# ModelTC/Dipoorlet

Hardware: AMD Instinct MI355X
Metric: calibration images/sec (whole node) + achieved HBM GB/s, ResNet-50 ONNX N=1024, -A hist (higher is better)
Workload: dtype f32; 1 GPU; ResNet-50 ONNX activation set (T=123, 26598376 fp32 elems/img), -A hist --bins 2048, N=1024 per GPU in 32 batches of 32: range pass + histogram pass + percentile clip; device=AMD Radeon Graphics (gfx950:sramecc+:xnack-), hist_checksum_ok=True, world_size_seen_by_backend=1

## Files before the change

### dipoorlet_amd/csrc/calib_kernels.hip

```cpp
#include "common.hpp"

#pragma clang fp contract(off)

namespace {

struct MinMaxOp {
    float mn, mx;
    uint32_t nan;
    __device__ __forceinline__ void operator()(float x) {
        mn = fminf(mn, x);
        mx = fmaxf(mx, x);
        nan |= (x != x);
    }
};

__device__ __forceinline__ void minmax_commit(const MinMaxOp& op, uint32_t slot, float* s_mn, float* s_mx, uint32_t* s_nan,
                                              uint32_t* __restrict__ min_enc, uint32_t* __restrict__ max_enc,
                                              uint32_t* __restrict__ nan_flag) {
    float mn = wave_min(op.mn), mx = wave_max(op.mx);
    uint32_t nn = __any(op.nan) ? 1u : 0u;
    const int w = threadIdx.x / kWave;
    if ((threadIdx.x & (kWave - 1)) == 0) {
        s_mn[w] = mn;
        s_mx[w] = mx;
        s_nan[w] = nn;
    }
    __syncthreads();
    if (threadIdx.x == 0) {
#pragma unroll
        for (int j = 1; j < kBlock / kWave; ++j) {
            mn = fminf(mn, s_mn[j]);
            mx = fmaxf(mx, s_mx[j]);
            nn |= s_nan[j];
        }
        if (mn <= mx) {
            atomicMin(min_enc + slot, enc_f32(mn));
            atomicMax(max_enc + slot, enc_f32(mx));
        }
        if (nn) atomicOr(nan_flag + slot, 1u);
    }
    __syncthreads();
}

__global__ __launch_bounds__(kBlock) void k_minmax(const dpl_work_item* __restrict__ items,
                                                    const uint32_t* __restrict__ bb,
                                                    const float* const* __restrict__ segs,
                                                    uint32_t* __restrict__ min_enc, uint32_t* __restrict__ max_enc,
                                                    uint32_t* __restrict__ nan_flag) {
    __shared__ float s_mn[kBlock / kWave], s_mx[kBlock / kWave];
    __shared__ uint32_t s_nan[kBlock / kWave];
    uint32_t k0, k1;
    block_items(bb, k0, k1);
    for (uint32_t k = k0; k < k1; ++k) {
        const dpl_work_item it = items[k];
        MinMaxOp op{INFINITY, -INFINITY, 0u};
        stream_span(segs[it.seg] + it.offset, it.count, op);
        minmax_commit(op, it.slot, s_mn, s_mx, s_nan, min_enc, max_enc, nan_flag);
    }
}

__global__ void k_minmax_init(uint32_t* mn, uint32_t* mx, uint32_t* nan, int64_t n) {
    int64_t i = (int64_t)blockIdx.x * blockDim.x + threadIdx.x;
    if (i < n) {
        mn[i] = 0xFFFFFFFFu;
        mx[i] = 0u;
        nan[i] = 0u;
    }
}

__device__ __forceinline__ void minmax_decode(uint32_t mn, uint32_t mx, uint32_t nan, float& omn, float& omx) {
    const bool bad = nan != 0u || mn == 0xFFFFFFFFu;
    omn = bad ? NAN : dec_f32(mn);
    omx = bad ? NAN : dec_f32(mx);
}

__global__ void k_minmax_finalize(const uint32_t* mn, const uint32_t* mx, const uint32_t* nan, int64_t n,
                                  float* omn, float* omx) {
    int64_t i = (int64_t)blockIdx.x * blockDim.x + threadIdx.x;
    if (i < n) minmax_decode(mn[i], mx[i], nan[i], omn[i], omx[i]);
}

__global__ void k_minmax_encode(const float* mn, const float* mx, int64_t n, uint32_t* emn, uint32_t* emx,
                                uint32_t* nan) {
    int64_t i = (int64_t)blockIdx.x * blockDim.x + threadIdx.x;
    if (i < n) {
        const bool bad = (mn[i] != mn[i]) || (mx[i] != mx[i]);
        emn[i] = bad ? 0xFFFFFFFFu : enc_f32(mn[i]);
        emx[i] = bad ? 0u : enc_f32(mx[i]);
        nan[i] = bad ? 1u : 0u;
    }
}

__device__ __forceinline__ float hist_edge(int i, float step, float first) {
    return __fadd_rn(__fmul_rn((float)i, step), first);
}

template <bool kFast>
struct HistOp {
    uint32_t* lds;
    float first, last, step, inv, denom;
    int last_bin;
    float fbins;
    uint32_t nonzero;
    __device__ __forceinline__ void operator()(float x) {
        const float a = fabsf(x);
        const bool nz = (a != 0.0f);
        nonzero += nz;
        if (kFast) {
            if (nz && (a <= last)) {
                const int i = (int)__fmul_rn(a, inv);
                const uint32_t dec = (a < __fmul_rn((float)i, step)) ? 0xFFFFFFFCu : 0u;
                atomicAdd(reinterpret_cast<uint32_t*>(reinterpret_cast<char*>(lds) + (((uint32_t)i << 2) + dec)), 1u);
            }
            return;
        }
        int i;
        if (kFast) {
            i = (int)__fmul_rn(a, inv);
            i = i > last_bin ? last_bin : i;
            i -= (a < __fmul_rn((float)i, step)) ? 1 : 0;
        } else {
            i = (int)__fmul_rn(__fdiv_rn(__fsub_rn(a, first), denom), fbins);
            i = i > last_bin ? last_bin : i;
            i = i < 0 ? 0 : i;
            i -= (a < hist_edge(i, step, first)) ? 1 : 0;
            i += (i != last_bin && a >= hist_edge(i + 1, step, first)) ? 1 : 0;
        }
        if (nz && (a <= last)) atomicAdd(lds + i, 1u);
    }
};

template <bool kFast>
__device__ __forceinline__ void hist_op_init(HistOp<kFast>& op, const dpl_hist_range& r, int bins, uint32_t* lds) {
    op.lds = lds;
    op.first = r.first;
    op.last = r.last;
    op.step = r.step;
    op.inv = r.inv;
    op.denom = __fsub_rn(r.last, r.first);
    op.last_bin = bins - 1;
    op.fbins = (float)bins;
    op.nonzero = 0u;
}

template <class Count>
__device__ __forceinline__ void hist_flush(uint32_t nonzero, const dpl_work_item& it, const dpl_hist_range& r, int bins,
                                           Count* __restrict__ hist, uint32_t* lds, uint32_t* s_nz) {
    const uint32_t nzw = wave_sum(nonzero);
    if ((threadIdx.x & (kWave - 1)) == 0) s_nz[threadIdx.x / kWave] = nzw;
    __syncthreads();
    if (threadIdx.x == 0) {
        uint32_t nzb = 0;
        for (int k = 0; k < kBlock / kWave; ++k) nzb += s_nz[k];
        const uint32_t z = it.count - nzb;
        if (z) atomicAdd(lds + r.zero_bin, z);
        const uint32_t top = lds[bins];
        if (top) atomicAdd(lds + bins - 1, top);
    }
    __syncthreads();
    Count* __restrict__ out = hist + (uint64_t)it.slot * (uint64_t)bins;
    for (int b = threadIdx.x; b < bins; b += kBlock) {
        const uint32_t c = lds[b];
        if (c) {
            if constexpr (sizeof(Count) == 8)
                atomicAdd(reinterpret_cast<unsigned long long*>(out + b), (unsigned long long)c);
            else
                atomicAdd(out + b, c);
        }
    }
}

template <bool kFast>
__device__ __forceinline__ void hist_body(const dpl_work_item& it, const float* const* __restrict__ segs,
                                          const dpl_hist_range& r, int bins, uint64_t* __restrict__ hist,
                                          uint32_t* lds, uint32_t* s_nz) {
    HistOp<kFast> op;
    hist_op_init(op, r, bins, lds);
    stream_span(segs[it.seg] + it.offset, it.count, op);
    hist_flush(op.nonzero, it, r, bins, hist, lds, s_nz);
}

__global__ __launch_bounds__(kBlock) void k_abs_hist(const dpl_work_item* __restrict__ items,
                                                      const uint32_t* __restrict__ bb,
                                                      const float* const* __restrict__ segs,
                                                      const dpl_hist_range* __restrict__ ranges, int bins,
                                                      uint64_t* __restrict__ hist) {
    extern __shared__ __attribute__((aligned(16))) uint32_t lds[];
    uint32_t* s_nz = lds + bins + 1;
    uint32_t k0, k1;
    block_items(bb, k0, k1);
    for (uint32_t k = k0; k < k1; ++k) {
        const dpl_work_item it = items[k];
        const dpl_hist_range r = ranges[it.slot];
        if (r.status != 0u) continue;
        for (int b = threadIdx.x; b <= bins; b += kBlock) lds[b] = 0u;
        __syncthreads();
        if (r.exact_div)
            hist_body<false>(it, segs, r, bins, hist, lds, s_nz);
        else
            hist_body<true>(it, segs, r, bins, hist, lds, s_nz);
        __syncthreads();
    }
}

__device__ __forceinline__ float py_max(float a, float b) { return (b > a) ? b : a; }
__device__ __forceinline__ float py_min(float a, float b) { return (b < a) ? b : a; }

__device__ __forceinline__ dpl_hist_range hist_range_of(float gmin, float gmax, int bins) {
    dpl_hist_range r;
    const float dmax = py_max(gmax, -gmin);
    float first = 0.0f, last = dmax;
    r.dmax = dmax;
    r.status = 0u;
    if (!(fabsf(last) <= 3.402823466e+38f) || last < first) r.status = 1u;
    if (first == last) {
        first = -0.5f;
        last = 0.5f;
    }
    const float delta = __fsub_rn(last, first);
    const float fb = (float)bins;
    r.first = first;
    r.last = last;
    r.step = __fdiv_rn(delta, fb);
    r.inv = __fmul_rn(__fdiv_rn(fb, delta), 1.000001f);
    if (r.status == 0u) {
        const float e1 = hist_edge(1, r.step, first);
        const float el = hist_edge(bins - 1, r.step, first);
        const float el2 = hist_edge(bins - 2 > 0 ? bins - 2 : 0, r.step, first);
        if (!(r.step > 0.0f) || !(e1 > first) || !(last > el) || (bins > 2 && !(el > el2))) r.status = 2u;
    }
    r.exact_div = (first != 0.0f || !(fabsf(r.inv) <= 3.402823466e+38f) || r.step < 1.0e-30f) ? 1u : 0u;
    {
        const float a = 0.0f;
        float t = __fmul_rn(__fdiv_rn(__fsub_rn(a, first), delta), fb);
        int b = (int)t;
        b = b > bins - 1 ? bins - 1 : b;
        b = b < 0 ? 0 : b;
        if (a < hist_edge(b, r.step, first)) --b;
        if (b != bins - 1 && a >= hist_edge(b + 1, r.step, first)) ++b;
        r.zero_bin = (uint32_t)(b < 0 ? 0 : b);
    }
    return r;
}

__global__ void k_hist_prepare(const float* __restrict__ gmin, const float* __restrict__ gmax, int64_t n, int bins,
                               dpl_hist_range* __restrict__ out) {
    int64_t i = (int64_t)blockIdx.x * blockDim.x + threadIdx.x;
    if (i >= n) return;
    out[i] = hist_range_of(gmin[i], gmax[i], bins);
}

__host__ __device__ inline uint64_t spec_counts_offset(int64_t n_slots) {
    return (((uint64_t)n_slots * (sizeof(dpl_hist_range) + sizeof(uint32_t))) + 15ull) & ~15ull;
}

__global__ __launch_bounds__(kBlock) void k_hist_snapshot(const uint32_t* __restrict__ mn, const uint32_t* __restrict__ mx,
                                                           const uint32_t* __restrict__ nan, int64_t n, int bins,
                                                           dpl_hist_range* __restrict__ snap, uint32_t* __restrict__ flags,
                                                           uint32_t* __restrict__ counts) {
    const int64_t i = (int64_t)blockIdx.x * blockDim.x + threadIdx.x;
    const int64_t stride = (int64_t)gridDim.x * blockDim.x;
    if (i < n) {
        float gmin, gmax;
        minmax_decode(mn[i], mx[i], nan[i], gmin, gmax);
        snap[i] = hist_range_of(gmin, gmax, bins);
        flags[i] = 0u;
    }
    const int64_t total = n * (int64_t)bins;
    for (int64_t j = i; j < total; j += stride) counts[j] = 0u;
}

template <bool kFast>
struct MinMaxHistOp {
    MinMaxOp m;
    HistOp<kFast> h;
    __device__ __forceinline__ void operator()(float x) {
        m(x);
        h(x);
    }
};

template <bool kFast>
__device__ __forceinline__ void minmax_hist_body(const dpl_work_item& it, const float* const* __restrict__ segs,
                                                 const dpl_hist_range& r, int bins, uint32_t* __restrict__ counts,
                                                 uint32_t* lds, uint32_t* s_nz, MinMaxOp& m) {
    MinMaxHistOp<kFast> op;
    op.m = m;
    hist_op_init(op.h, r, bins, lds);
    stream_span(segs[it.seg] + it.offset, it.count, op);
    m = op.m;
    hist_flush(op.h.nonzero, it, r, bins, counts, lds, s_nz);
}

__global__ __launch_bounds__(kBlock) void k_minmax_hist(const dpl_work_item* __restrict__ items,
                                                         const uint32_t* __restrict__ bb,
                                                         const float* const* __restrict__ segs,
                                                         uint32_t* __restrict__ min_enc, uint32_t* __restrict__ max_enc,
                                                         uint32_t* __restrict__ nan_flag,
                                                         const dpl_hist_range* __restrict__ snap, int bins,
                                                         uint32_t* __restrict__ counts) {
    extern __shared__ __attribute__((aligned(16))) uint32_t lds_mh[];
    uint32_t* s_nz = lds_mh + bins + 1;
    float* s_mn = reinterpret_cast<float*>(s_nz + kBlock / kWave);
    float* s_mx = s_mn + kBlock / kWave;
    uint32_t* s_nan = reinterpret_cast<uint32_t*>(s_mx + kBlock / kWave);
    uint32_t k0, k1;
    block_items(bb, k0, k1);
    for (uint32_t k = k0; k < k1; ++k) {
        const dpl_work_item it = items[k];
        const dpl_hist_range r = snap[it.slot];
        MinMaxOp m{INFINITY, -INFINITY, 0u};
        if (r.status != 0u) {
            stream_span(segs[it.seg] + it.offset, it.count, m);
        } else {
            for (int b = threadIdx.x; b <= bins; b += kBlock) lds_mh[b] = 0u;
            __syncthreads();
            if (r.exact_div)
                minmax_hist_body<false>(it, segs, r, bins, counts, lds_mh, s_nz, m);
            else
                minmax_hist_body<true>(it, segs, r, bins, counts, lds_mh, s_nz, m);
        }
        minmax_commit(m, it.slot, s_mn, s_mx, s_nan, min_enc, max_enc, nan_flag);
    }
}

__global__ __launch_bounds__(kBlock) void k_hist_resolve(const dpl_hist_range* __restrict__ snap,
                                                          const dpl_hist_range* __restrict__ fin,
                                                          const uint32_t* __restrict__ counts, const uint64_t* __restrict__ elems,
                                                          int bins, uint64_t* __restrict__ hist, uint32_t* __restrict__ flags,
                                                          unsigned long long* __restrict__ stats) {
    const uint32_t t = blockIdx.x;
    const uint32_t* a = reinterpret_cast<const uint32_t*>(snap + t);
    const uint32_t* b = reinterpret_cast<const uint32_t*>(fin + t);
    bool same = true;
#pragma unroll
    for (int w = 0; w < (int)(sizeof(dpl_hist_range) / 4); ++w) same = same && (a[w] == b[w]);
    const uint32_t status = fin[t].status;
    const bool valid = same && status == 0u;
    if (threadIdx.x == 0) {
        flags[t] = valid ? 1u : (status != 0u ? 2u : 0u);
        if (stats) {
            const unsigned long long e = elems[t];
            atomicAdd(stats + 0, 1ull);
            atomicAdd(stats + 2, e);
            if (valid) {
                atomicAdd(stats + 1, 1ull);
                atomicAdd(stats + 3, e);
            }
        }
    }
    if (!valid) return;
    const uint32_t* __restrict__ row = counts + (uint64_t)t * (uint64_t)bins;
    uint64_t* __restrict__ out = hist + (uint64_t)t * (uint64_t)bins;
    for (int j = threadIdx.x; j < bins; j += kBlock) {
        const uint32_t c = row[j];
        if (c) out[j] += (uint64_t)c;
    }
}

__device__ __forceinline__ uint64_t shfl_up_u64(uint64_t v, int d) {
    const uint32_t lo = __shfl_up((uint32_t)v, d, kWave), hi = __shfl_up((uint32_t)(v >> 32), d, kWave);
    return ((uint64_t)hi << 32) | lo;
}

__device__ __forceinline__ void rest_prefix(const uint64_t* __restrict__ elems, const uint32_t* __restrict__ flags, int n_tensors,
                                            uint64_t* P, uint64_t* s_tot) {
    const int per = (n_tensors + kBlock - 1) / kBlock;
    const int t0 = (int)threadIdx.x * per;
    uint64_t mine = 0;
    for (int j = 0; j < per; ++j) {
        const int t = t0 + j;
        if (t < n_tensors && flags[t] == 0u) mine += elems[t];
    }
    uint64_t incl = mine;
    const int lane = threadIdx.x & (kWave - 1), wv = threadIdx.x / kWave;
#pragma unroll
    for (int o = 1; o < kWave; o <<= 1) {
        const uint64_t up = shfl_up_u64(incl, o);
        if (lane >= o) incl += up;
    }
    if (lane == kWave - 1) s_tot[wv] = incl;
    __syncthreads();
    uint64_t run = incl - mine;
    for (int w = 0; w < wv; ++w) run += s_tot[w];
    for (int j = 0; j < per; ++j) {
        const int t = t0 + j;
        if (t < n_tensors) {
            P[t] = run;
            if (flags[t] == 0u) run += elems[t];
        }
    }
    if (threadIdx.x == kBlock - 1) P[n_tensors] = run;
    __syncthreads();
}

__device__ __forceinline__ void rest_cut(const uint64_t* P, int n_tensors, uint64_t G, uint64_t b, uint64_t& cut, int& at) {
    const uint64_t total = P[n_tensors], q = total / G, rem = total % G;
    const uint64_t target = (b >= G) ? total : q * b + (rem * b) / G;
    if (target >= total) {
        cut = total;
        at = n_tensors;
        return;
    }
    int lo = 1, hi = n_tensors;
    while (lo < hi) {
        const int mid = (lo + hi) >> 1;
        if (P[mid] > target) hi = mid; else lo = mid + 1;
    }
    at = lo - 1;
    cut = P[lo - 1] + ((target - P[lo - 1]) & ~1023ull);
}

__global__ __launch_bounds__(kBlock) void k_abs_hist_rest(const uint64_t* __restrict__ elems, const uint32_t* __restrict__ flags,
                                                           int n_tensors, const float* const* __restrict__ segs,
                                                           const dpl_hist_range* __restrict__ ranges, int bins,
                                                           uint64_t* __restrict__ hist) {
    extern __shared__ __attribute__((aligned(16))) uint32_t lds_rest[];
    uint64_t* P = reinterpret_cast<uint64_t*>(lds_rest);
    uint64_t* s_tot = P + n_tensors + 1;
    uint32_t* lds = reinterpret_cast<uint32_t*>(s_tot + kBlock / kWave);
    uint32_t* s_nz = lds + bins + 1;
    rest_prefix(elems, flags, n_tensors, P, s_tot);
    if (P[n_tensors] == 0) return;
    uint64_t cut[2];
    int at[2];
    rest_cut(P, n_tensors, gridDim.x, blockIdx.x, cut[0], at[0]);
    rest_cut(P, n_tensors, gridDim.x, (uint64_t)blockIdx.x + 1, cut[1], at[1]);
    uint64_t pos = cut[0];
    const uint64_t end = cut[1];
    int t = at[0];
    while (pos < end) {
        while (P[t + 1] <= pos) ++t;
        const uint64_t stop = P[t + 1] < end ? P[t + 1] : end;
        dpl_work_item it;
        it.offset = pos - P[t];
        it.count = (uint32_t)(stop - pos);
        it.seg = (uint32_t)t;
        it.slot = (uint32_t)t;
        it.reserved = 0u;
        const dpl_hist_range r = ranges[t];
        for (int b = threadIdx.x; b <= bins; b += kBlock) lds[b] = 0u;
        __syncthreads();
        if (r.exact_div)
            hist_body<false>(it, segs, r, bins, hist, lds, s_nz);
        else
            hist_body<true>(it, segs, r, bins, hist, lds, s_nz);
        __syncthreads();
        pos = stop;
    }
}

__global__ __launch_bounds__(kBlock) void k_hist_spec_cuts(const uint64_t* __restrict__ elems, const uint32_t* __restrict__ flags,
                                                            int n_tensors, uint64_t* __restrict__ cuts) {
    extern __shared__ __attribute__((aligned(16))) uint32_t lds_cuts[];
    uint64_t* P = reinterpret_cast<uint64_t*>(lds_cuts);
    uint64_t* s_tot = P + n_tensors + 1;
    rest_prefix(elems, flags, n_tensors, P, s_tot);
    if (threadIdx.x != 0) return;
    uint64_t cut = 0;
    int at = 0;
    if (P[n_tensors] != 0) rest_cut(P, n_tensors, gridDim.x, blockIdx.x, cut, at);
    cuts[blockIdx.x] = cut;
    if (blockIdx.x + 1 == gridDim.x) cuts[gridDim.x] = P[n_tensors];
}

__device__ __forceinline__ void store_bin_clip(int found, float gmin, float gmax, int bins, float* __restrict__ clip) {
    float lo = gmin, hi = gmax;
    if (found >= 0) {
        const float dmax = py_max(-gmin, gmax);
        const float cv = __fmul_rn((float)found + 0.5f, __fdiv_rn(dmax, (float)bins));
        lo = py_max(-cv, gmin);
        hi = py_min(cv, gmax);
    }
    clip[0] = lo;
    clip[1] = hi;
}

__global__ __launch_bounds__(kWave) void k_hist_percentile(const uint64_t* __restrict__ hist,
                                                            const float* __restrict__ gmin_a,
                                                            const float* __restrict__ gmax_a, int bins,
                                                            double threshold, float* __restrict__ clip) {
    const int slot = blockIdx.x;
    const int lane = threadIdx.x;
    const uint64_t* h = hist + (uint64_t)slot * bins;
    unsigned long long tot = 0;
    for (int b = lane; b < bins; b += kWave) tot += h[b];
#pragma unroll
    for (int o = 32; o > 0; o >>= 1) tot += __shfl_xor(tot, o, kWave);
    const double total = (double)(long long)tot;
    const float gmin = gmin_a[slot], gmax = gmax_a[slot];
    double accum = 0.0;
    int found = -1;
    uint64_t raw_next = lane < bins ? h[lane] : 0ull;
    for (int base = 0; base < bins && found < 0; base += kWave) {
        const int b = base + lane;
        const double hv = (b < bins) ? (double)(float)(long long)raw_next / total : 0.0;
        raw_next = (b + kWave < bins) ? h[b + kWave] : 0ull;
        const int lim = (bins - base) < kWave ? (bins - base) : kWave;
        const int h_lo = __double2loint(hv), h_hi = __double2hiint(hv);
        uint64_t reached = 0;
        if (lim == kWave) {
#pragma unroll
            for (int j = 0; j < kWave; ++j) {
                accum += __hiloint2double(__builtin_amdgcn_readlane(h_hi, j), __builtin_amdgcn_readlane(h_lo, j));
                reached |= (accum >= threshold) ? (1ull << j) : 0ull;
// ... 122 lines not shown
    for (int o = 32; o > 0; o >>= 1) {
        const double ov = __shfl_xor(bv, o, kWave);
        const int oi = __shfl_xor(bi, o, kWave);
        if (ov < bv || (ov == bv && oi >= 0 && (bi < 0 || oi < bi))) {
            bv = ov;
            bi = oi;
        }
    }
    if (lane == 0) {
        best[slot] = bi;
        store_bin_clip(bi >= 0 ? bi - 1 : -1, gmin_a[slot], gmax_a[slot], bins, clip + 2 * slot);
    }
}

constexpr int kGridUniform = DPL_GRID_UNIFORM, kGridE4M3 = DPL_GRID_E4M3;

template <int GRID>
__global__ __launch_bounds__(kBlock) void k_hist_qmse(const uint64_t* __restrict__ hist, int bins, int first, int top, int n_chunks,
                                                       double* __restrict__ err) {
    extern __shared__ __attribute__((aligned(16))) double qm_lds[];
    double* hd = qm_lds;
    uint64_t* part = reinterpret_cast<uint64_t*>(hd + bins);
    const uint32_t tid = threadIdx.x, lane = tid & (kWave - 1), wave = tid / kWave;
    const uint32_t slot = blockIdx.x / (uint32_t)n_chunks, chunk = blockIdx.x % (uint32_t)n_chunks;
    const uint64_t* __restrict__ h = hist + (uint64_t)slot * (uint64_t)bins;
    double* __restrict__ out = err + (uint64_t)slot * ((uint64_t)bins + 1u);
    const uint32_t F = (uint32_t)first, C = (uint32_t)n_chunks, nb = (uint32_t)bins;

    uint64_t s = 0;
    for (uint32_t b = tid; b < nb; b += kBlock) {
        const uint64_t v = h[b];
        s += v;
        hd[b] = (double)(long long)v;
    }
#pragma unroll
    for (int o = 32; o > 0; o >>= 1) s += __shfl_xor(s, o, kWave);
    if (lane == 0) part[wave] = s;
    __syncthreads();
    uint64_t N = 0;
#pragma unroll
    for (int w = 0; w < kBlock / kWave; ++w) N += part[w];

    for (uint32_t i = chunk + tid * C; i < F; i += kBlock * C) out[i] = INFINITY;

    constexpr double unit = GRID == kGridE4M3 ? 512.0 : 1.0;
    const double dtop = GRID == kGridE4M3 ? 448.0 : (double)top;
    const double atop = unit * dtop;
    const double norm = (double)(long long)N * (4.0 * atop * atop);
    for (uint32_t i = F + chunk + wave * C; i <= nb; i += (kBlock / kWave) * C) {
        const double t = (double)(2u * i - 1u);
        const double rt = 1.0 / (unit * t);
        double acc = 0.0;
        if (N != 0ull) {
            for (uint32_t b = lane; b < nb; b += kWave) {
                const double hb = hd[b];
                if (hb != 0.0) {
                    const double a = (double)(2u * b + 1u) * atop;
                    const double v = fmin(a * rt, dtop);
                    double q;
                    if (GRID == kGridE4M3) {
                        int e = (int)((__double_as_longlong(v) >> 52) & 0x7FF) - 1023;
                        e = e < -6 ? -6 : e;
                        const double istep = __longlong_as_double((long long)(1023 + 3 - e) << 52);
                        const double step512 = __longlong_as_double((long long)(1023 + 9 - 3 + e) << 52);
                        q = rint(v * istep) * step512;
                    } else {
                        q = rint(v);
                    }
                    const double dt = a - q * t;
                    acc += hb * (dt * dt);
                }
            }
            acc = wave_sum(acc);
        }
        if (lane == 0) out[i] = N != 0ull ? acc / norm : INFINITY;
    }
}

__global__ __launch_bounds__(kBlock) void k_rowwise_minmax(const float* __restrict__ w, int64_t cols,
                                                            float* __restrict__ omn, float* __restrict__ omx) {
    __shared__ float s_mn[kBlock / kWave], s_mx[kBlock / kWave];
    __shared__ uint32_t s_nan[kBlock / kWave];
    const float* p = w + (int64_t)blockIdx.x * cols;
    MinMaxOp op{INFINITY, -INFINITY, 0u};
    stream_span(p, (uint32_t)cols, op);
    float mn = wave_min(op.mn), mx = wave_max(op.mx);
    uint32_t nn = __any(op.nan) ? 1u : 0u;
    const int wv = threadIdx.x / kWave;
    if ((threadIdx.x & (kWave - 1)) == 0) {
        s_mn[wv] = mn;
        s_mx[wv] = mx;
        s_nan[wv] = nn;
    }
    __syncthreads();
    if (threadIdx.x == 0) {
        for (int k = 1; k < kBlock / kWave; ++k) {
            mn = fminf(mn, s_mn[k]);
            mx = fmaxf(mx, s_mx[k]);
            nn |= s_nan[k];
        }
        omn[blockIdx.x] = nn ? NAN : mn;
        omx[blockIdx.x] = nn ? NAN : mx;
    }
}

constexpr int kColMaxLanes = 64;
constexpr int kColUnroll = 4;
constexpr int kColMaxBlocks = 2048;
using u4 = __attribute__((ext_vector_type(4))) uint32_t;

template <class T>
__global__ __launch_bounds__(kBlock) void k_colwise_absmax(const T* __restrict__ x_generic, uint64_t rows, uint64_t cv, uint32_t tw,
                                                            uint32_t* __restrict__ acc) {
    __shared__ T s_m[kBlock];
    const __attribute__((address_space(1))) T* x = (const __attribute__((address_space(1))) T*)x_generic;
    const uint32_t tid = threadIdx.x, rp = kBlock / tw;
    const uint64_t c = (uint64_t)blockIdx.x * tw + (tid & (tw - 1));
    T m = T(0);
    if (c < cv) {
        const uint64_t step = (uint64_t)gridDim.y * rp;
        for (uint64_t r = (uint64_t)blockIdx.y * rp + tid / tw; r < rows; r += kColUnroll * step) {
            T v[kColUnroll];
#pragma unroll
            for (int u = 0; u < kColUnroll; ++u) {
                const uint64_t rr = r + u * step;
                v[u] = __builtin_nontemporal_load(x + (rr < rows ? rr : rows - 1) * cv + c);
            }
#pragma unroll
            for (int u = 0; u < kColUnroll; ++u) m = __builtin_elementwise_max(m, v[u] & T(0x7FFFFFFFu));
        }
    }
    s_m[tid] = m;
    __syncthreads();
    for (uint32_t h = kBlock / 2; h >= tw; h >>= 1) {
        if (tid < h) s_m[tid] = __builtin_elementwise_max(s_m[tid], s_m[tid + h]);
        __syncthreads();
    }
    if (tid < tw && c < cv) {
        m = s_m[tid];
        if constexpr (sizeof(T) == 16) {
            uint32_t* a = acc + 4 * c;
            const uint32_t a0 = a[0], a1 = a[1], a2 = a[2], a3 = a[3];
            if (m.x > a0) atomicMax(a + 0, m.x);
            if (m.y > a1) atomicMax(a + 1, m.y);
            if (m.z > a2) atomicMax(a + 2, m.z);
            if (m.w > a3) atomicMax(a + 3, m.w);
        } else {
            if (m > acc[c]) atomicMax(acc + c, m);
        }
    }
}

__device__ __forceinline__ float fq_one(float x, float scale, float zp, float qlo, float qhi) {
    float q = __fadd_rn(rintf(__fdiv_rn(x, scale)), zp);
    q = fminf(fmaxf(q, qlo), qhi);
    return __fmul_rn(__fsub_rn(q, zp), scale);
}

__device__ __forceinline__ float e4m3_round(float v) {
    const float a = fminf(fabsf(v), 448.f);
    uint32_t e = __float_as_uint(a) >> 23;
    e = e < 121u ? 121u : e;
    const float step = __uint_as_float((e - 3u) << 23), inv = __uint_as_float((257u - e) << 23);
    const float r = copysignf(__fmul_rn(rintf(__fmul_rn(a, inv)), step), v);
    return v != v ? v : r;
}

enum { kFqFmtInt = 0, kFqFmtE4M3 = 1 };
template <int FMT>
__device__ __forceinline__ float fq_elem(float x, float scale, float zp, float qlo, float qhi) {
// ... 525 lines not shown
}

int dpl_minmax_finalize(const uint32_t* d_min_enc, const uint32_t* d_max_enc, const uint32_t* d_nan,
                        int64_t n_slots, float* d_min, float* d_max, dpl_stream_t s) {
    if (n_slots <= 0) return 0;
    hipLaunchKernelGGL(k_minmax_finalize, dim3(grid_for(n_slots, 256)), dim3(256), 0, (hipStream_t)s, d_min_enc,
                       d_max_enc, d_nan, n_slots, d_min, d_max);
    DPL_LAUNCH_CHECK("k_minmax_finalize");
    return 0;
}

int dpl_minmax_encode(const float* d_min, const float* d_max, int64_t n_slots, uint32_t* d_min_enc,
                      uint32_t* d_max_enc, uint32_t* d_nan, dpl_stream_t s) {
    if (n_slots <= 0) return 0;
    hipLaunchKernelGGL(k_minmax_encode, dim3(grid_for(n_slots, 256)), dim3(256), 0, (hipStream_t)s, d_min, d_max,
                       n_slots, d_min_enc, d_max_enc, d_nan);
    DPL_LAUNCH_CHECK("k_minmax_encode");
    return 0;
}

int dpl_hist_prepare(const float* d_min, const float* d_max, int64_t n_slots, int bins, dpl_hist_range* d_ranges,
                     dpl_stream_t s) {
    if (bins < 1 || bins > DPL_MAX_BINS) return fail_msg("dpl_hist_prepare: bins must be in [1, 16384]");
    if (n_slots <= 0) return 0;
    hipLaunchKernelGGL(k_hist_prepare, dim3(grid_for(n_slots, 64)), dim3(64), 0, (hipStream_t)s, d_min, d_max,
                       n_slots, bins, d_ranges);
    DPL_LAUNCH_CHECK("k_hist_prepare");
    return 0;
}

int dpl_abs_hist_accumulate(const dpl_work_item* d_items, int64_t n_items, const uint32_t* d_block_begin,
                            int64_t n_blocks, const float* const* d_seg_ptrs, const dpl_hist_range* d_ranges,
                            int bins, uint64_t* d_hist, dpl_stream_t s) {
    if (bins < 1 || bins > DPL_MAX_BINS) return fail_msg("dpl_abs_hist_accumulate: bins must be in [1, 16384]");
    if (n_items <= 0) return 0;
    if (int e = check_blocks("dpl_abs_hist_accumulate", n_items, d_block_begin, n_blocks)) return e;
    hipLaunchKernelGGL(k_abs_hist, dim3((unsigned)n_blocks), dim3(kBlock),
                       ((size_t)bins + 1 + kBlock / kWave) * sizeof(uint32_t), (hipStream_t)s, d_items, d_block_begin,
                       d_seg_ptrs, d_ranges, bins, d_hist);
    DPL_LAUNCH_CHECK("k_abs_hist");
    return 0;
}

uint64_t dpl_hist_spec_entry_bytes(int64_t n_slots, int bins) {
    if (n_slots < 0 || bins < 1 || bins > DPL_MAX_BINS) return 0;
    return spec_counts_offset(n_slots) + (uint64_t)n_slots * (uint64_t)bins * sizeof(uint32_t);
}

int dpl_minmax_hist_accumulate(const dpl_work_item* d_items, int64_t n_items, const uint32_t* d_block_begin,
                               int64_t n_blocks, const float* const* d_seg_ptrs, uint32_t* d_min_enc, uint32_t* d_max_enc,
                               uint32_t* d_nan, int64_t n_slots, int bins, void* d_entry, dpl_stream_t s) {
    if (bins < 1 || bins > DPL_MAX_BINS) return fail_msg("dpl_minmax_hist_accumulate: bins must be in [1, 16384]");
    if (!d_entry || ((uintptr_t)d_entry & 15u)) return fail_msg("dpl_minmax_hist_accumulate: d_entry must be 16-byte aligned");
    if (n_slots <= 0 || n_slots > 0x7FFFFFFFll) return fail_msg("dpl_minmax_hist_accumulate: n_slots out of range");
    if (n_items <= 0) return 0;
    if (int e = check_blocks("dpl_minmax_hist_accumulate", n_items, d_block_begin, n_blocks)) return e;
    dpl_hist_range* snap = (dpl_hist_range*)d_entry;
    uint32_t* flags = (uint32_t*)(snap + n_slots);
    uint32_t* counts = (uint32_t*)((char*)d_entry + spec_counts_offset(n_slots));
    int64_t zb = grid_for(n_slots * (int64_t)bins, kBlock * 8);
    if (zb < grid_for(n_slots, kBlock)) zb = grid_for(n_slots, kBlock);
    if (zb > 1024) zb = 1024;
    hipLaunchKernelGGL(k_hist_snapshot, dim3((unsigned)zb), dim3(kBlock), 0, (hipStream_t)s, d_min_enc, d_max_enc, d_nan,
                       n_slots, bins, snap, flags, counts);
    DPL_LAUNCH_CHECK("k_hist_snapshot");
    hipLaunchKernelGGL(k_minmax_hist, dim3((unsigned)n_blocks), dim3(kBlock),
                       ((size_t)bins + 1 + 4 * (kBlock / kWave)) * sizeof(uint32_t), (hipStream_t)s, d_items, d_block_begin,
                       d_seg_ptrs, d_min_enc, d_max_enc, d_nan, snap, bins, counts);
    DPL_LAUNCH_CHECK("k_minmax_hist");
    return 0;
}

int dpl_hist_spec_accumulate(void* d_entry, const uint64_t* d_elems, int64_t n_slots, int64_t n_blocks,
                             const float* const* d_seg_ptrs, const dpl_hist_range* d_ranges, int bins, uint64_t* d_hist,
                             uint64_t* d_stats, dpl_stream_t s) {
    if (bins < 1 || bins > DPL_MAX_BINS) return fail_msg("dpl_hist_spec_accumulate: bins must be in [1, 16384]");
    if (!d_entry || ((uintptr_t)d_entry & 15u)) return fail_msg("dpl_hist_spec_accumulate: d_entry must be 16-byte aligned");
    if (n_slots <= 0 || n_slots > DPL_HIST_SPEC_MAX_TENSORS)
        return fail_msg("dpl_hist_spec_accumulate: n_slots must be in [1, DPL_HIST_SPEC_MAX_TENSORS]");
    if (n_blocks <= 0 || n_blocks > 0x7FFFFFFFll) return fail_msg("dpl_hist_spec_accumulate: n_blocks out of range");
    dpl_hist_range* snap = (dpl_hist_range*)d_entry;
    uint32_t* flags = (uint32_t*)(snap + n_slots);
    const uint32_t* counts = (const uint32_t*)((char*)d_entry + spec_counts_offset(n_slots));
    hipLaunchKernelGGL(k_hist_resolve, dim3((unsigned)n_slots), dim3(kBlock), 0, (hipStream_t)s, snap, d_ranges, counts, d_elems,
                       bins, d_hist, flags, (unsigned long long*)d_stats);
    DPL_LAUNCH_CHECK("k_hist_resolve");
    const size_t lds = ((size_t)n_slots + 1 + kBlock / kWave) * sizeof(uint64_t) + ((size_t)bins + 1 + kBlock / kWave) * sizeof(uint32_t);
    hipLaunchKernelGGL(k_abs_hist_rest, dim3((unsigned)n_blocks), dim3(kBlock), lds, (hipStream_t)s, d_elems, flags, (int)n_slots,
                       d_seg_ptrs, d_ranges, bins, d_hist);
    DPL_LAUNCH_CHECK("k_abs_hist_rest");
    return 0;
}

int dpl_hist_spec_cuts(const void* d_entry, const uint64_t* d_elems, int64_t n_slots, int64_t n_blocks, uint64_t* d_cuts,
                       dpl_stream_t s) {
    if (!d_entry || !d_cuts) return fail_msg("dpl_hist_spec_cuts: null argument");
    if (n_slots <= 0 || n_slots > DPL_HIST_SPEC_MAX_TENSORS)
        return fail_msg("dpl_hist_spec_cuts: n_slots must be in [1, DPL_HIST_SPEC_MAX_TENSORS]");
    if (n_blocks <= 0 || n_blocks > 0x7FFFFFFFll) return fail_msg("dpl_hist_spec_cuts: n_blocks out of range");
    const uint32_t* flags = (const uint32_t*)((const dpl_hist_range*)d_entry + n_slots);
    hipLaunchKernelGGL(k_hist_spec_cuts, dim3((unsigned)n_blocks), dim3(kBlock),
                       ((size_t)n_slots + 1 + kBlock / kWave) * sizeof(uint64_t), (hipStream_t)s, d_elems, flags, (int)n_slots, d_cuts);
    DPL_LAUNCH_CHECK("k_hist_spec_cuts");
    return 0;
}

int dpl_hist_percentile(const uint64_t* d_hist, const float* d_min, const float* d_max, int64_t n_slots, int bins,
                        double threshold, float* d_clip, dpl_stream_t s) {
    if (n_slots <= 0) return 0;
    hipLaunchKernelGGL(k_hist_percentile, dim3((unsigned)n_slots), dim3(kWave), 0, (hipStream_t)s, d_hist, d_min,
                       d_max, bins, threshold, d_clip);
    DPL_LAUNCH_CHECK("k_hist_percentile");
    return 0;
}

int dpl_hist_kl(const uint64_t* d_hist, const float* d_min, const float* d_max, int64_t n_slots, int bins, int levels,
                double* d_div, int32_t* d_best, float* d_clip, dpl_stream_t s) {
    if (bins < 1 || bins > DPL_MAX_BINS) return fail_msg("dpl_hist_kl: bins must be in [1, 16384]");
    if (levels < 2 || levels > bins) return fail_msg("dpl_hist_kl: levels must be in [2, bins]");
    if (n_slots <= 0) return 0;
    const int64_t n_cand = (int64_t)bins - levels + 1;
    int64_t chunks = (1024 + n_slots - 1) / n_slots;
    if (chunks > n_cand / 8) chunks = n_cand / 8;
    if (chunks < 1) chunks = 1;
    if (n_slots * chunks > 0x7FFFFFFFll) return fail_msg("dpl_hist_kl: too many slots");
    const size_t nblk = ((size_t)bins + 63) / 64;
    const size_t lds = ((size_t)bins + 1 + nblk + 1 + kBlock) * sizeof(uint64_t) + (nblk + 1) * sizeof(uint32_t);
    hipLaunchKernelGGL(k_hist_kl, dim3((unsigned)(n_slots * chunks)), dim3(kBlock), lds, (hipStream_t)s, d_hist, bins, levels,
                       (int)chunks, d_div);
    DPL_LAUNCH_CHECK("k_hist_kl");
    hipLaunchKernelGGL(k_hist_kl_pick, dim3((unsigned)n_slots), dim3(kWave), 0, (hipStream_t)s, d_div, d_min, d_max, bins,
                       d_best, d_clip);
    DPL_LAUNCH_CHECK("k_hist_kl_pick");
    return 0;
}

int dpl_hist_qmse(const uint64_t* d_hist, const float* d_min, const float* d_max, int64_t n_slots, int bins, int first, int grid,
                  int top, double* d_err, int32_t* d_best, float* d_clip, dpl_stream_t s) {
    if (bins < 1 || bins > DPL_MAX_BINS) return fail_msg("dpl_hist_qmse: bins must be in [1, 16384]");
    if (first < 1 || first > bins) return fail_msg("dpl_hist_qmse: first must be in [1, bins]");
    if (grid != DPL_GRID_UNIFORM && grid != DPL_GRID_E4M3) return fail_msg("dpl_hist_qmse: grid must be DPL_GRID_UNIFORM or DPL_GRID_E4M3");
    if (grid == DPL_GRID_UNIFORM && (top < 1 || top > 32767)) return fail_msg("dpl_hist_qmse: top must be in [1, 32767] on the uniform grid");
    if (grid == DPL_GRID_E4M3 && top != 0) return fail_msg("dpl_hist_qmse: top must be 0 on the E4M3 grid (its largest value is 448)");
    if (n_slots <= 0) return 0;
    const int64_t n_cand = (int64_t)bins - first + 1;
    int64_t chunks = (1024 + n_slots - 1) / n_slots;
    if (chunks > n_cand / 8) chunks = n_cand / 8;
    if (chunks < 1) chunks = 1;
    if (n_slots * chunks > 0x7FFFFFFFll) return fail_msg("dpl_hist_qmse: too many slots");
    const size_t lds = (size_t)bins * sizeof(double) + (kBlock / kWave) * sizeof(uint64_t);
    const dim3 wgs((unsigned)(n_slots * chunks));
    if (grid == DPL_GRID_E4M3)
        hipLaunchKernelGGL(k_hist_qmse<kGridE4M3>, wgs, dim3(kBlock), lds, (hipStream_t)s, d_hist, bins, first, top, (int)chunks, d_err);
    else
        hipLaunchKernelGGL(k_hist_qmse<kGridUniform>, wgs, dim3(kBlock), lds, (hipStream_t)s, d_hist, bins, first, top, (int)chunks, d_err);
    DPL_LAUNCH_CHECK("k_hist_qmse");
    hipLaunchKernelGGL(k_hist_kl_pick, dim3((unsigned)n_slots), dim3(kWave), 0, (hipStream_t)s, d_err, d_min, d_max, bins,
                       d_best, d_clip);
    DPL_LAUNCH_CHECK("k_hist_kl_pick");
    return 0;
}

int dpl_rowwise_minmax(const float* d_w, int64_t rows, int64_t cols, float* d_min, float* d_max, dpl_stream_t s) {
    if (rows <= 0) return 0;
    if (cols <= 0 || cols > 0xFFFFFFFFll) return fail_msg("dpl_rowwise_minmax: cols out of range");
    hipLaunchKernelGGL(k_rowwise_minmax, dim3((unsigned)rows), dim3(kBlock), 0, (hipStream_t)s, d_w, cols, d_min,
                       d_max);
    DPL_LAUNCH_CHECK("k_rowwise_minmax");
    return 0;
}

int dpl_colwise_absmax(const float* d_x, int64_t rows, int64_t cols, float* d_acc, dpl_stream_t s) {
    if (rows < 0 || cols < 1) return fail_msg("dpl_colwise_absmax: rows must be >= 0 and cols >= 1");
// ... 100 lines not shown
```

### dipoorlet_amd/csrc/common.hpp

```cpp
#pragma once
#include <hip/hip_runtime.h>
#include <stdint.h>
#include <string.h>
#include <stdio.h>
#include <math.h>
#include <stdlib.h>

#include "../../include/dipoorlet_hip.h"

#pragma clang fp contract(off)

namespace dpl {
inline thread_local char g_err[512] = "";
}

namespace {

using dpl::g_err;
constexpr int kBlock = 256;
constexpr int kUnroll = 4;
constexpr int kWave = 64;
using f4 = __attribute__((ext_vector_type(4))) float;

int fail(const char* what, hipError_t e) {
    snprintf(g_err, sizeof(g_err), "%s: %s", what, hipGetErrorString(e));
    return -1;
}
int fail_msg(const char* what) {
    snprintf(g_err, sizeof(g_err), "%s", what);
    return -2;
}
#define DPL_LAUNCH_CHECK(name)                              \
    do {                                                    \
        hipError_t e__ = hipGetLastError();                 \
        if (e__ != hipSuccess) return fail(name, e__);      \
    } while (0)

__host__ __device__ inline uint32_t enc_f32(float f) {
    uint32_t b;
    memcpy(&b, &f, 4);
    return b ^ ((b >> 31) ? 0xFFFFFFFFu : 0x80000000u);
}
__host__ __device__ inline float dec_f32(uint32_t u) {
    uint32_t b = u ^ ((u >> 31) ? 0x80000000u : 0xFFFFFFFFu);
    float f;
    memcpy(&f, &b, 4);
    return f;
}

__device__ __forceinline__ float wave_min(float v) {
#pragma unroll
    for (int o = 32; o > 0; o >>= 1) v = fminf(v, __shfl_xor(v, o, kWave));
    return v;
}
__device__ __forceinline__ float wave_max(float v) {
#pragma unroll
    for (int o = 32; o > 0; o >>= 1) v = fmaxf(v, __shfl_xor(v, o, kWave));
    return v;
}
__device__ __forceinline__ double wave_sum(double v) {
#pragma unroll
    for (int o = 32; o > 0; o >>= 1) v += __shfl_xor(v, o, kWave);
    return v;
}
__device__ __forceinline__ uint32_t wave_sum(uint32_t v) {
#pragma unroll
    for (int o = 32; o > 0; o >>= 1) v += __shfl_xor(v, o, kWave);
    return v;
}

typedef const __attribute__((address_space(1))) f4* gptr_f4;
typedef const __attribute__((address_space(1))) float* gptr_f32;

template <class Op>
__device__ __forceinline__ void stream_span(const float* __restrict__ p_generic, uint32_t n, Op& op) {
    const uint32_t tid = threadIdx.x;
    gptr_f32 p = (gptr_f32)p_generic;
    uint32_t head = (uint32_t)(((16u - (uint32_t)((uintptr_t)p_generic & 15u)) & 15u) >> 2);
    if (head > n) head = n;
    if (tid < head) op(p[tid]);
    p += head;
    n -= head;
    const uint32_t nvec = n >> 2;
    gptr_f4 pv = (gptr_f4)p;
    uint32_t i = tid;
    constexpr uint32_t kStride = kUnroll * kBlock;
#define DPL_LOAD(buf, base)                                                                       \
    _Pragma("unroll") for (int u = 0; u < kUnroll; ++u) buf[u] = __builtin_nontemporal_load(pv + (base) + u * kBlock)
#define DPL_EAT(buf)                                 \
    _Pragma("unroll") for (int u = 0; u < kUnroll; ++u) { \
        op(buf[u].x);                                \
        op(buf[u].y);                                \
        op(buf[u].z);                                \
        op(buf[u].w);                                \
    }
    if (i + (kUnroll - 1) * kBlock < nvec) {
        f4 A[kUnroll], B[kUnroll];
        DPL_LOAD(A, i);
        i += kStride;
        for (;;) {
            if (!(i + (kUnroll - 1) * kBlock < nvec)) {
                DPL_EAT(A);
                break;
            }
            DPL_LOAD(B, i);
            i += kStride;
            DPL_EAT(A);
            if (!(i + (kUnroll - 1) * kBlock < nvec)) {
                DPL_EAT(B);
                break;
            }
            DPL_LOAD(A, i);
            i += kStride;
            DPL_EAT(B);
        }
    }
#undef DPL_LOAD
#undef DPL_EAT
    for (; i < nvec; i += kBlock) {
        f4 v = __builtin_nontemporal_load(pv + i);
        op(v.x);
        op(v.y);
        op(v.z);
        op(v.w);
    }
    const uint32_t t = (nvec << 2) + tid;
    if (t < n) op(p[t]);
}

__device__ __forceinline__ void block_items(const uint32_t* __restrict__ bb, uint32_t& k0, uint32_t& k1) {
    if (bb) {
        k0 = bb[blockIdx.x];
        k1 = bb[blockIdx.x + 1];
    } else {
        k0 = blockIdx.x;
        k1 = k0 + 1;
    }
}

inline int grid_for(int64_t n, int per_block) { return (int)((n + per_block - 1) / per_block); }

inline int check_blocks(const char* who, int64_t n_items, const uint32_t* d_block_begin, int64_t n_blocks) {
    if (n_blocks <= 0 || n_blocks > 0x7FFFFFFFll || (!d_block_begin && n_blocks != n_items)) {
        snprintf(g_err, sizeof(g_err), "%s: n_blocks must be positive and equal n_items when d_block_begin is null", who);
        return -2;
    }
    return 0;
}

}
```

Measured before the change: 57410 images/s.

## Use wave-ballot NaN/nonzero counting, wave-uniform stream loop, and fuse hist resolve into rest kernel

MinMaxOp now accumulates NaN flags as a 64-bit wave ballot, and a vec() path checks two elements per unordered compare. HistOp counts nonzeros with a ballot popcount, which drops the wave_sum reduction at flush. stream_span makes the unrolled loop condition wave-uniform through readfirstlane when the op has vec(), aiming to keep branches scalar. The separate k_hist_resolve launch is merged into a new k_hist_spec kernel that computes flags in LDS, merges speculative rows with a batched load/store, and then runs the rest pass. This removes one kernel launch and its per-tensor blocks, at the cost of more LDS use and the same row merge work spread over fewer blocks.

```diff
diff --git a/dipoorlet_amd/csrc/calib_kernels.hip b/dipoorlet_amd/csrc/calib_kernels.hip
--- a/dipoorlet_amd/csrc/calib_kernels.hip
+++ b/dipoorlet_amd/csrc/calib_kernels.hip
@@ -6,11 +6,23 @@
 
 struct MinMaxOp {
     float mn, mx;
-    uint32_t nan;
+    uint64_t nan;
     __device__ __forceinline__ void operator()(float x) {
         mn = fminf(mn, x);
         mx = fmaxf(mx, x);
-        nan |= (x != x);
+        nan |= __builtin_amdgcn_ballot_w64(__builtin_isunordered(x, x));
+    }
+    __device__ __forceinline__ void vec(const f4& v) {
+        mn = fminf(mn, v.x);
+        mx = fmaxf(mx, v.x);
+        mn = fminf(mn, v.y);
+        mx = fmaxf(mx, v.y);
+        mn = fminf(mn, v.z);
+        mx = fmaxf(mx, v.z);
+        mn = fminf(mn, v.w);
+        mx = fmaxf(mx, v.w);
+        nan |= __builtin_amdgcn_ballot_w64(__builtin_isunordered(v.x, v.y));
+        nan |= __builtin_amdgcn_ballot_w64(__builtin_isunordered(v.z, v.w));
     }
 };
 
@@ -18,7 +30,7 @@
                                               uint32_t* __restrict__ min_enc, uint32_t* __restrict__ max_enc,
                                               uint32_t* __restrict__ nan_flag) {
     float mn = wave_min(op.mn), mx = wave_max(op.mx);
-    uint32_t nn = __any(op.nan) ? 1u : 0u;
+    uint32_t nn = op.nan != 0ull ? 1u : 0u;
     const int w = threadIdx.x / kWave;
     if ((threadIdx.x & (kWave - 1)) == 0) {
         s_mn[w] = mn;
@@ -53,7 +65,7 @@
     block_items(bb, k0, k1);
     for (uint32_t k = k0; k < k1; ++k) {
         const dpl_work_item it = items[k];
-        MinMaxOp op{INFINITY, -INFINITY, 0u};
+        MinMaxOp op{INFINITY, -INFINITY, 0ull};
         stream_span(segs[it.seg] + it.offset, it.count, op);
         minmax_commit(op, it.slot, s_mn, s_mx, s_nan, min_enc, max_enc, nan_flag);
     }
@@ -102,10 +114,16 @@
     int last_bin;
     float fbins;
     uint32_t nonzero;
+    __device__ __forceinline__ void vec(const f4& v) {
+        (*this)(v.x);
+        (*this)(v.y);
+        (*this)(v.z);
+        (*this)(v.w);
+    }
     __device__ __forceinline__ void operator()(float x) {
         const float a = fabsf(x);
         const bool nz = (a != 0.0f);
-        nonzero += nz;
+        nonzero += (uint32_t)__builtin_popcountll(__builtin_amdgcn_ballot_w64(nz));
         if (kFast) {
             if (nz && (a <= last)) {
                 const int i = (int)__fmul_rn(a, inv);
@@ -146,8 +164,7 @@
 template <class Count>
 __device__ __forceinline__ void hist_flush(uint32_t nonzero, const dpl_work_item& it, const dpl_hist_range& r, int bins,
                                            Count* __restrict__ hist, uint32_t* lds, uint32_t* s_nz) {
-    const uint32_t nzw = wave_sum(nonzero);
-    if ((threadIdx.x & (kWave - 1)) == 0) s_nz[threadIdx.x / kWave] = nzw;
+    if ((threadIdx.x & (kWave - 1)) == 0) s_nz[threadIdx.x / kWave] = nonzero;
     __syncthreads();
     if (threadIdx.x == 0) {
         uint32_t nzb = 0;
@@ -278,6 +295,10 @@
         m(x);
         h(x);
     }
+    __device__ __forceinline__ void vec(const f4& v) {
+        m.vec(v);
+        h.vec(v);
+    }
 };
 
 template <bool kFast>
@@ -309,7 +330,7 @@
     for (uint32_t k = k0; k < k1; ++k) {
         const dpl_work_item it = items[k];
         const dpl_hist_range r = snap[it.slot];
-        MinMaxOp m{INFINITY, -INFINITY, 0u};
+        MinMaxOp m{INFINITY, -INFINITY, 0ull};
         if (r.status != 0u) {
             stream_span(segs[it.seg] + it.offset, it.count, m);
         } else {
@@ -324,38 +345,15 @@
     }
 }
 
-__global__ __launch_bounds__(kBlock) void k_hist_resolve(const dpl_hist_range* __restrict__ snap,
-                                                          const dpl_hist_range* __restrict__ fin,
-                                                          const uint32_t* __restrict__ counts, const uint64_t* __restrict__ elems,
-                                                          int bins, uint64_t* __restrict__ hist, uint32_t* __restrict__ flags,
-                                                          unsigned long long* __restrict__ stats) {
-    const uint32_t t = blockIdx.x;
+__device__ __forceinline__ uint32_t spec_flag_of(const dpl_hist_range* __restrict__ snap, const dpl_hist_range* __restrict__ fin,
+                                                 uint32_t t) {
     const uint32_t* a = reinterpret_cast<const uint32_t*>(snap + t);
     const uint32_t* b = reinterpret_cast<const uint32_t*>(fin + t);
     bool same = true;
 #pragma unroll
     for (int w = 0; w < (int)(sizeof(dpl_hist_range) / 4); ++w) same = same && (a[w] == b[w]);
     const uint32_t status = fin[t].status;
-    const bool valid = same && status == 0u;
-    if (threadIdx.x == 0) {
-        flags[t] = valid ? 1u : (status != 0u ? 2u : 0u);
-        if (stats) {
-            const unsigned long long e = elems[t];
-            atomicAdd(stats + 0, 1ull);
-            atomicAdd(stats + 2, e);
-            if (valid) {
-                atomicAdd(stats + 1, 1ull);
-                atomicAdd(stats + 3, e);
-            }
-        }
-    }
-    if (!valid) return;
-    const uint32_t* __restrict__ row = counts + (uint64_t)t * (uint64_t)bins;
-    uint64_t* __restrict__ out = hist + (uint64_t)t * (uint64_t)bins;
-    for (int j = threadIdx.x; j < bins; j += kBlock) {
-        const uint32_t c = row[j];
-        if (c) out[j] += (uint64_t)c;
-    }
+    return (same && status == 0u) ? 1u : (status != 0u ? 2u : 0u);
 }
 
 __device__ __forceinline__ uint64_t shfl_up_u64(uint64_t v, int d) {
@@ -411,16 +409,58 @@
     cut = P[lo - 1] + ((target - P[lo - 1]) & ~1023ull);
 }
 
-__global__ __launch_bounds__(kBlock) void k_abs_hist_rest(const uint64_t* __restrict__ elems, const uint32_t* __restrict__ flags,
-                                                           int n_tensors, const float* const* __restrict__ segs,
-                                                           const dpl_hist_range* __restrict__ ranges, int bins,
-                                                           uint64_t* __restrict__ hist) {
+constexpr size_t hist_spec_lds(size_t n_tensors, size_t bins) {
+    return (n_tensors + 1 + kBlock / kWave) * sizeof(uint64_t) + (bins + 1 + kBlock / kWave) * sizeof(uint32_t) + n_tensors * sizeof(uint32_t);
+}
+static_assert(hist_spec_lds(DPL_HIST_SPEC_MAX_TENSORS, DPL_MAX_BINS) <= 160u * 1024u, "k_hist_spec's LDS must fit a workgroup's 160 KiB");
+constexpr int kRowTrip = 8;
+
+__global__ __launch_bounds__(kBlock) void k_hist_spec(const dpl_hist_range* __restrict__ snap,
+                                                       const dpl_hist_range* __restrict__ ranges,
+                                                       const uint32_t* __restrict__ counts, const uint64_t* __restrict__ elems,
+                                                       int n_tensors, const float* const* __restrict__ segs, int bins,
+                                                       uint64_t* __restrict__ hist, uint32_t* __restrict__ flags,
+                                                       unsigned long long* __restrict__ stats) {
     extern __shared__ __attribute__((aligned(16))) uint32_t lds_rest[];
     uint64_t* P = reinterpret_cast<uint64_t*>(lds_rest);
     uint64_t* s_tot = P + n_tensors + 1;
     uint32_t* lds = reinterpret_cast<uint32_t*>(s_tot + kBlock / kWave);
     uint32_t* s_nz = lds + bins + 1;
-    rest_prefix(elems, flags, n_tensors, P, s_tot);
+    uint32_t* s_flag = s_nz + kBlock / kWave;
+    for (int t = threadIdx.x; t < n_tensors; t += kBlock) s_flag[t] = spec_flag_of(snap, ranges, (uint32_t)t);
+    __syncthreads();
+    for (uint32_t t = blockIdx.x; t < (uint32_t)n_tensors; t += gridDim.x) {
+        const uint32_t f = s_flag[t];
+        if (threadIdx.x == 0) {
+            flags[t] = f;
+            if (stats) {
+                const unsigned long long e = elems[t];
+                atomicAdd(stats + 0, 1ull);
+                atomicAdd(stats + 2, e);
+                if (f == 1u) {
+                    atomicAdd(stats + 1, 1ull);
+                    atomicAdd(stats + 3, e);
+                }
+            }
+        }
+        if (f != 1u) continue;
+        const uint32_t* __restrict__ row = counts + (uint64_t)t * (uint64_t)bins;
+        uint64_t* __restrict__ out = hist + (uint64_t)t * (uint64_t)bins;
+        for (int j0 = threadIdx.x; j0 < bins; j0 += kRowTrip * kBlock) {
+            uint32_t c[kRowTrip];
+            uint64_t h[kRowTrip];
+#pragma unroll
+            for (int u = 0; u < kRowTrip; ++u) {
+                const int j = j0 + u * kBlock;
+                c[u] = j < bins ? row[j] : 0u;
+                h[u] = j < bins ? out[j] : 0ull;
+            }
+#pragma unroll
+            for (int u = 0; u < kRowTrip; ++u)
+                if (c[u]) out[j0 + u * kBlock] = h[u] + (uint64_t)c[u];
+        }
+    }
+    rest_prefix(elems, s_flag, n_tensors, P, s_tot);
     if (P[n_tensors] == 0) return;
     uint64_t cut[2];
     int at[2];
@@ -709,10 +749,10 @@
     __shared__ float s_mn[kBlock / kWave], s_mx[kBlock / kWave];
     __shared__ uint32_t s_nan[kBlock / kWave];
     const float* p = w + (int64_t)blockIdx.x * cols;
-    MinMaxOp op{INFINITY, -INFINITY, 0u};
+    MinMaxOp op{INFINITY, -INFINITY, 0ull};
     stream_span(p, (uint32_t)cols, op);
     float mn = wave_min(op.mn), mx = wave_max(op.mx);
-    uint32_t nn = __any(op.nan) ? 1u : 0u;
+    uint32_t nn = op.nan != 0ull ? 1u : 0u;
     const int wv = threadIdx.x / kWave;
     if ((threadIdx.x & (kWave - 1)) == 0) {
         s_mn[wv] = mn;
@@ -1404,13 +1444,9 @@
     dpl_hist_range* snap = (dpl_hist_range*)d_entry;
     uint32_t* flags = (uint32_t*)(snap + n_slots);
     const uint32_t* counts = (const uint32_t*)((char*)d_entry + spec_counts_offset(n_slots));
-    hipLaunchKernelGGL(k_hist_resolve, dim3((unsigned)n_slots), dim3(kBlock), 0, (hipStream_t)s, snap, d_ranges, counts, d_elems,
-                       bins, d_hist, flags, (unsigned long long*)d_stats);
-    DPL_LAUNCH_CHECK("k_hist_resolve");
-    const size_t lds = ((size_t)n_slots + 1 + kBlock / kWave) * sizeof(uint64_t) + ((size_t)bins + 1 + kBlock / kWave) * sizeof(uint32_t);
-    hipLaunchKernelGGL(k_abs_hist_rest, dim3((unsigned)n_blocks), dim3(kBlock), lds, (hipStream_t)s, d_elems, flags, (int)n_slots,
-                       d_seg_ptrs, d_ranges, bins, d_hist);
-    DPL_LAUNCH_CHECK("k_abs_hist_rest");
+    hipLaunchKernelGGL(k_hist_spec, dim3((unsigned)n_blocks), dim3(kBlock), hist_spec_lds((size_t)n_slots, (size_t)bins), (hipStream_t)s,
+                       snap, d_ranges, counts, d_elems, (int)n_slots, d_seg_ptrs, bins, d_hist, flags, (unsigned long long*)d_stats);
+    DPL_LAUNCH_CHECK("k_hist_spec");
     return 0;
 }
 
diff --git a/dipoorlet_amd/csrc/common.hpp b/dipoorlet_amd/csrc/common.hpp
--- a/dipoorlet_amd/csrc/common.hpp
+++ b/dipoorlet_amd/csrc/common.hpp
@@ -5,6 +5,8 @@
 #include <stdio.h>
 #include <math.h>
 #include <stdlib.h>
+#include <type_traits>
+#include <utility>
 
 #include "../../include/dipoorlet_hip.h"
 
@@ -72,6 +74,23 @@
 typedef const __attribute__((address_space(1))) f4* gptr_f4;
 typedef const __attribute__((address_space(1))) float* gptr_f32;
 
+template <class Op, class = void>
+struct op_has_vec : std::false_type {};
+template <class Op>
+struct op_has_vec<Op, std::void_t<decltype(std::declval<Op&>().vec(std::declval<const f4&>()))>> : std::true_type {};
+
+template <class Op>
+__device__ __forceinline__ void stream_eat(Op& op, const f4& v) {
+    if constexpr (op_has_vec<Op>::value) {
+        op.vec(v);
+    } else {
+        op(v.x);
+        op(v.y);
+        op(v.z);
+        op(v.w);
+    }
+}
+
 template <class Op>
 __device__ __forceinline__ void stream_span(const float* __restrict__ p_generic, uint32_t n, Op& op) {
     const uint32_t tid = threadIdx.x;
@@ -84,34 +103,32 @@
     const uint32_t nvec = n >> 2;
     gptr_f4 pv = (gptr_f4)p;
     uint32_t i = tid;
+    uint32_t il = op_has_vec<Op>::value ? (uint32_t)__builtin_amdgcn_readfirstlane((int)(tid | (kWave - 1))) : tid;
     constexpr uint32_t kStride = kUnroll * kBlock;
 #define DPL_LOAD(buf, base)                                                                       \
     _Pragma("unroll") for (int u = 0; u < kUnroll; ++u) buf[u] = __builtin_nontemporal_load(pv + (base) + u * kBlock)
-#define DPL_EAT(buf)                                 \
-    _Pragma("unroll") for (int u = 0; u < kUnroll; ++u) { \
-        op(buf[u].x);                                \
-        op(buf[u].y);                                \
-        op(buf[u].z);                                \
-        op(buf[u].w);                                \
-    }
-    if (i + (kUnroll - 1) * kBlock < nvec) {
+#define DPL_EAT(buf) _Pragma("unroll") for (int u = 0; u < kUnroll; ++u) stream_eat(op, buf[u])
+    if (il + (kUnroll - 1) * kBlock < nvec) {
         f4 A[kUnroll], B[kUnroll];
         DPL_LOAD(A, i);
         i += kStride;
+        il += kStride;
         for (;;) {
-            if (!(i + (kUnroll - 1) * kBlock < nvec)) {
+            if (!(il + (kUnroll - 1) * kBlock < nvec)) {
                 DPL_EAT(A);
                 break;
             }
             DPL_LOAD(B, i);
             i += kStride;
+            il += kStride;
             DPL_EAT(A);
-            if (!(i + (kUnroll - 1) * kBlock < nvec)) {
+            if (!(il + (kUnroll - 1) * kBlock < nvec)) {
                 DPL_EAT(B);
                 break;
             }
             DPL_LOAD(A, i);
             i += kStride;
+            il += kStride;
             DPL_EAT(B);
         }
     }
@@ -119,10 +136,7 @@
 #undef DPL_EAT
     for (; i < nvec; i += kBlock) {
         f4 v = __builtin_nontemporal_load(pv + i);
-        op(v.x);
-        op(v.y);
-        op(v.z);
-        op(v.w);
+        stream_eat(op, v);
     }
     const uint32_t t = (nvec << 2) + tid;
     if (t < n) op(p[t]);
```

Measured after the change: 57670 images/s (median of 6 runs). No clear change (+0.5%).
